# goodmattg/ndivplanning

Hardware: AMD Instinct MI355X
Metric: gan_train_steps_per_sec_traj8_batch64 (higher is better)
Workload: dtype f32; 1 GPU; BASELINE configs[1]: train_gan.py step (D update + G update), codes mode, batch=64 trajectories per GPU, traj_len=8, num_sample=6, noise_dim=2; rows_per_gpu=2688, global_batch=64, parallelism=dp1, hip_graph=True, steps_per_graph_launch=16, repeats=1, gradient_exchange=none

## Files before the change

### ndivplanning_amd/csrc/ndp_kernels.hip

```cpp
#include <hip/hip_runtime.h>
#include <math.h>
#include <stddef.h>
#include <stdint.h>

#include "ndp_device.h"

namespace ndp {

#ifdef NDP_STAMPS
__device__ unsigned long long* g_stamps = nullptr;
__device__ int g_stamp_kernel = 0;
#define NDP_STAMP_ON(id) (g_stamps != nullptr && (g_stamp_kernel == 0 || g_stamp_kernel == (id)))
#define NDP_STAMP_DECL __shared__ unsigned long long stamp_store_[64]; unsigned long long* stamp_lds_ = stamp_store_
#define NDP_STAMP_PTR stamp_lds_
#define NDP_STAMP(i)                                             \
  do {                                                           \
    if (threadIdx.x == 0) {                                      \
      stamp_lds_[2 * (i)] = clock64();                           \
      stamp_lds_[2 * (i) + 1] = wall_clock64();                  \
    }                                                            \
  } while (0)
#define NDP_STAMP_FLUSH(n, id)                                                              \
  do {                                                                                      \
    if (threadIdx.x == 0 && NDP_STAMP_ON(id))                                               \
// ... 845 lines not shown
      if (row < a.m)
        if constexpr (WT) stg4_wt(a.action_hat + row0 * 4, 4 * threadIdx.x, *reinterpret_cast<const f32x4*>(A + threadIdx.x * 4));
        else *reinterpret_cast<f32x4*>(a.action_hat + row * 4) = *reinterpret_cast<const f32x4*>(A + threadIdx.x * 4);
    }
    __syncthreads();
    NDP_STAMP(9);
    phase_a_d_part<PK, RG, NR>(a, false, tile, ntiles, dw1, dw2, CPD, XC, XT, B1, B2, L, DL, W4S, NDP_STAMP_PTR);
  } else {
    const int tile = (int)blockIdx.x - ntiles;
    const int64_t row0 = (int64_t)tile * R;
    dw1.preload(PK ? d.pf1 : d.w1 + ADIM, 260, d.b1, d.w1, ADIM);
    W4S[threadIdx.x] = d.w4[threadIdx.x];
    if (threadIdx.x == 0) W4S[256] = d.b4[0];
    for (int idx = threadIdx.x; idx < R * 64; idx += kThreads) {
      const int i = idx >> 6, k = 4 * (idx & 63);
      const int64_t row = row0 + i;
      f32x4 v = {0.f, 0.f, 0.f, 0.f};
      if (row < a.flat) v = *reinterpret_cast<const f32x4*>(a.code + row * CODE + k);
      *reinterpret_cast<f32x4*>(XC + i * 260 + k) = v;
    }
    for (int idx = threadIdx.x; idx < R * TAILLD; idx += kThreads) {
      const int i = idx / TAILLD, t = idx % TAILLD;
      const int64_t row = row0 + i;
      XT[idx] = (row < a.flat && t < ADIM) ? a.actions[row * ADIM + t] : 0.f;
    }
    __syncthreads();
    phase_a_d_part<PK, RG, 0>(a, true, tile, ntiles, dw1, dw2, nullptr, XC, XT, B1, B2, L, DL, W4S, NDP_STAMP_PTR);
  }
  (void)red;
  NDP_STAMP(8);
  NDP_STAMP_FLUSH(32, 5);
}

struct PhaseBArgs {
  GNet g; DNet d;
  const float* code; int code_rep;
  const float* action_hat;
  const float* nd_grad;
  int64_t m;
  float inv_m;
  const float *gh1, *gh2, *gh3, *gh4;
  float *dy1, *dy2, *dy3, *dy4, *dy5;
  float* loss_partials;
  float* dy1seg; int seg_s, seg_entries;
};

constexpr int phase_b_lds_floats(bool pre) {
  return 16 * (260 + TAILLD + 132 + 68 + 132 + 4 + 2) + 8 + 256 + kSW4 + kSW5 + (pre ? 16 * (260 + 132 + 68) : 0);
}

template <bool PK, int RG, bool PRE, int NR>
__global__ __launch_bounds__(kThreads, (RG >= 96 ? 2 : 3)) void k_phase_b(PhaseBArgs a_segment) {
  constexpr bool DD = NR > 0;
  constexpr int NRR = NR > 0 ? NR : 1;
  constexpr bool WT = wt_tiles(RG);
  const PhaseBArgs a = RG >= 96 ? load_kernargs<PhaseBArgs>() : a_segment;
  constexpr int R = 16;
  extern __shared__ __attribute__((aligned(16))) float smem[];
  float* XC = smem;
  float* XT = XC + R * 260;
  float* B1 = XT + R * TAILLD;
  float* B2 = B1 + R * 132;
  float* H1 = B2 + R * 68;
  float* DA = H1 + R * 132;
  float* L = DA + R * 4;
  float* DL = L + R;
  float* red = DL + R;
  float* W1A = red + 8;
  float* W4S = W1A + 256;
  float* W5S = W4S + kSW4;
  float* G4 = PRE ? W5S + kSW5 : XC;
  float* G3 = PRE ? G4 + R * 260 : B1;
  float* G2 = PRE ? G3 + R * 132 : B2;
  const int64_t row0 = (int64_t)blockIdx.x * R;
  const GNet& g = a.g;
  const DNet& d = a.d;
  NDP_STAMP_DECL;
  NDP_STAMP(0);

  FwdW<256, 64, 4, PK, RG> dw1;
  FwdW<64, 128, 4, PK, RG> dw2;
  f32x4 ct[R * 64 / kThreads];
  float av = 0.f;
  {
    if (DD) {
      load_code_rows<NRR>(XC, a.code, row0 / a.code_rep, (a.m + a.code_rep - 1) / a.code_rep);
    } else {
#pragma unroll
      for (int u = 0; u < R * 64 / kThreads; ++u) {
        const int idx = threadIdx.x + u * kThreads;
        const int i = idx >> 6, k = 4 * (idx & 63);
        const int64_t row = row0 + i;
        const bool ok = row < a.m;
        const f32x4 v = *reinterpret_cast<const f32x4*>(a.code + ((ok ? row : 0) / a.code_rep) * CODE + k);
        ct[u] = ok ? v : f32x4{0.f, 0.f, 0.f, 0.f};
      }
    }
    const int i = threadIdx.x / TAILLD, t = threadIdx.x % TAILLD;
    const int64_t row = row0 + i;
    if (row < a.m && t < ADIM) av = a.action_hat[row * ADIM + t];
  }
  const float w1a = d.w1[(threadIdx.x >> 2) * 260 + (threadIdx.x & 3)], w4r = d.w4[threadIdx.x], b4r = d.b4[0];
  const f32x4 w5r = *reinterpret_cast<const f32x4*>(g.w5 + 4 * threadIdx.x);
  pin_vmem();
  if (DD) dw2.preload(PK ? d.pf2 : d.w2, 64, d.b2, nullptr, 0);
  else dw1.preload(PK ? d.pf1 : d.w1 + ADIM, 260, d.b1, d.w1, ADIM);
  if (!DD) {
#pragma unroll
    for (int u = 0; u < R * 64 / kThreads; ++u) {
      const int idx = threadIdx.x + u * kThreads;
      *reinterpret_cast<f32x4*>(XC + (idx >> 6) * 260 + 4 * (idx & 63)) = ct[u];
    }
  }
  XT[threadIdx.x] = av;
  TileRegs<1, 128> t1;
  TileRegs<1, 256> t4;
  TileRegs<1, 128> t3;
  TileRegs<1, 64> t2;
  W1A[threadIdx.x] = w1a;
  W4S[threadIdx.x] = w4r;
  if (threadIdx.x == 0) W4S[256] = b4r;
  *reinterpret_cast<f32x4*>(W5S + 4 * threadIdx.x) = w5r;
  if (PRE) {
    t1.load(a.gh1 + row0 * 128, 128);
    t4.load(a.gh4 + row0 * 256, 256);
    t3.load(a.gh3 + row0 * 128, 128);
    t2.load(a.gh2 + row0 * 64, 64);
    pin_vmem();
  } else {
    load_tile<1, 128>(H1, 132, a.gh1 + row0 * 128, 128);
  }
  __syncthreads();
  NDP_STAMP(1);
  if (DD) {
    code_rows_dot<64, NRR>(d.pf1, XC, XC + NRR * 260);
    __syncthreads();
    fc1_from_code_rows<64, ACT_LRELU, NRR>(XC + NRR * 260, d.b1, d.w1, 260, ADIM, XT, B2, 68,
                                           (int)(row0 % a.code_rep), a.code_rep);
  } else {
    dw2.bind(PK ? d.pf2 : d.w2, 64, d.b2, nullptr, 0);
    layer_fwd_run<1, 256, 64, ACT_LRELU, 4, PK>(dw1, XC, 260, B2, 68, XT, TAILLD, dw2);
  }
  if (PRE) {
    t1.store(H1, 132);
    t4.store(G4, 260);
    t3.store(G3, 132);
    t2.store(G2, 68);
  }
  __syncthreads();
  FwdW<128, 256, 4, PK, RG> dw3;
  dw3.bind(PK ? d.pf3 : d.w3, 128, d.b3, nullptr, 0);
  layer_fwd_run<1, 64, 128, ACT_LRELU, 4, PK>(dw2, B2, 68, B1, 132, nullptr, 0, dw3);
  __syncthreads();
  DgW<128, 256, PK, RG> dg3;
  dg3.bind(PK ? d.pg3 : d.w3, 128);
  layer_fwd_run<1, 128, 256, ACT_LRELU, 4, PK>(dw3, B1, 132, XC, 260, nullptr, 0, dg3);
  __syncthreads();
  NDP_STAMP(2);
  layer_fwd_narrow<1, 256, 1>(XC, 260, W4S, W4S + 256, L, 1);
  __syncthreads();
  float lsum = 0.f;
  if (threadIdx.x < R) {
    const int64_t row = row0 + threadIdx.x;
    const float x = L[threadIdx.x];
    float dl = 0.f;
    if (row < a.m) {
      lsum = fmaxf(x, 0.f) - x + log1pf(expf(-fabsf(x)));
      dl = (1.f / (1.f + expf(-x)) - 1.f) * a.inv_m;
    }
    DL[threadIdx.x] = dl;
  }
  if (threadIdx.x < 64) {
    const float tot = wave_sum(lsum);
    if (threadIdx.x == 0) a.loss_partials[blockIdx.x] = tot;
  }
  __syncthreads();
  NDP_STAMP(3);
  layer_dgrad_narrow<1, 256, 1, ACT_LRELU>(DL, 1, W4S, XC, 260);
  __syncthreads();
  DgW<64, 128, PK, RG> dg2;
  dg2.bind(PK ? d.pg2 : d.w2, 64);
  layer_dgrad_run<1, 128, 256, ACT_LRELU, PK>(dg3, XC, 260, B1, 132, dg2);
  __syncthreads();
  DgW<128, 256, PK, RG> gg4;
  gg4.bind(PK ? g.pg4 : g.w4, 128);
  layer_dgrad_run<1, 64, 128, ACT_LRELU, PK>(dg2, B1, 132, B2, 68, gg4);
  __syncthreads();
  NDP_STAMP(4);
  {
    const int i = threadIdx.x >> 4, j = (threadIdx.x >> 2) & 3, part = threadIdx.x & 3;
    const int64_t row = row0 + i;
    const float ng = (part == 0 && row < a.m && a.nd_grad != nullptr) ? a.nd_grad[row * ADIM + j] : 0.f;
    float s = 0.f;
#pragma unroll
    for (int o = 16 * part; o < 16 * part + 16; ++o) s = fmaf(B2[i * 68 + o], W1A[o * 4 + j], s);
    s += __shfl_xor(s, 1, 64);
    s += __shfl_xor(s, 2, 64);
    if (part == 0) {
      s = row < a.m ? s + ng : 0.f;
      DA[i * ADIM + j] = s;
      a.dy5[row * ADIM + j] = s;
    }
  }
  __syncthreads();
  NDP_STAMP(5);

  if (!PRE) {
    load_tile<1, 256>(G4, 260, a.gh4 + row0 * 256, 256);
    load_tile<1, 128>(G3, 132, a.gh3 + row0 * 128, 128);
    load_tile<1, 64>(G2, 68, a.gh2 + row0 * 64, 64);
    __syncthreads();
  }
  NDP_STAMP(6);
  layer_dgrad_narrow<1, 256, 4, ACT_RELU>(DA, 4, W5S, G4, 260);
  __syncthreads();
  NDP_STAMP(7);
  DgW<64, 128, PK, RG> gg3;
  gg3.bind(PK ? g.pg3 : g.w3, 64);
  layer_dgrad_run<1, 128, 256, ACT_RELU, PK>(gg4, G4, 260, G3, 132, gg3);
  __syncthreads();
  NDP_STAMP(8);
  DgW<128, 64, PK, RG> gg2;
  gg2.bind(PK ? g.pg2 : g.w2, 128);
  store_tile<1, 256, WT>(a.dy4 + row0 * 256, 256, G4, 260);
  layer_dgrad_run<1, 64, 128, ACT_RELU, PK>(gg3, G3, 132, G2, 68, gg2);
  __syncthreads();
  NDP_STAMP(9);
  store_tile<1, 128, WT>(a.dy3 + row0 * 128, 128, G3, 132);
  layer_dgrad_run<1, 128, 64, ACT_RELU, PK>(gg2, G2, 68, H1, 132);
  __syncthreads();
  NDP_STAMP(10);
  store_tile<1, 64, WT>(a.dy2 + row0 * 64, 64, G2, 68);
  store_tile<1, 128, WT>(a.dy1 + row0 * 128, 128, H1, 132);
  store_segment_sums<128, 1>(H1, 132, a.dy1seg, row0, a.code_rep, a.seg_s, a.seg_entries, (int)blockIdx.x, (int)gridDim.x);
  NDP_STAMP(11);
  NDP_STAMP_FLUSH(12, 6);
}

__device__ __forceinline__ void adam_advance(int32_t* state, float lr, float b1, float b2) {
  const int32_t t = state[0] + 1;
  state[0] = t;
  const double bc1 = 1.0 - pow((double)b1, (double)t);
  const double bc2 = 1.0 - pow((double)b2, (double)t);
  reinterpret_cast<float*>(state)[1] = (float)((double)lr / bc1);
  reinterpret_cast<float*>(state)[2] = (float)sqrt(bc2);
}

enum { WG_FULL = 0, WG_SKINNY_B = 1, WG_SKINNY_A = 2, WG_WIDE = 3 };
constexpr int kWgradPrefetch = 8;

struct WgradJob {
  const float* A;
  const float* B;
  int lda, ldb;
  int a_cols, b_cols;
  int b_rowmod, b_rowdiv, b_rowmax;
  int b_vec;
  int dst_off, dst_ld;
  int bias_off;
  int kind;
  int rows, seg, seg_s, seg_k;
  int seg_wrap;
  int nchunks;
};
constexpr int kMaxJobs = 28;
struct WgradHead {
  int njobs;
  int nwide;
  int wide_chunks;
  int rows;
  float* slabs;
  int64_t slab_stride;
  int32_t* bump;
  float lr, beta1, beta2;
  int nchunks;
  NdivArgs nd;
};
struct WgradArgs : WgradHead {
  WgradJob job[kMaxJobs];
  int net_is_g;
  int nreg, reg_begin[4], reg_end[4];
  int wide_begin, wide_end;
};

__host__ __device__ __forceinline__ void wgrad_slot(int njobs, int nwide, int wide_chunks, int block, int& job, int& chunk) {
  const int wide_blocks = nwide * wide_chunks;
  if (block < wide_blocks) {
    job = njobs + block / wide_chunks;
    chunk = block % wide_chunks;
  } else {
    const int b = block - wide_blocks;
    const int idx = b >> 3;
    job = idx % njobs;
    chunk = (b & 7) + 8 * (idx / njobs);
  }
}

#ifdef NDP_STAMPS
#define NDP_WSTAMP(i) do { if (threadIdx.x == 0) { wst[2 * (i)] = clock64(); wst[2 * (i) + 1] = wall_clock64(); } } while (0)
#else
#define NDP_WSTAMP(i) do { } while (0)
#endif

template <int MT, int NT, int KIND, bool WT>
__device__ __forceinline__ void wgrad_block(const WgradJob& jb, int rbeg, int rend, int row_last,
                                            float* slab, float* smem, unsigned long long* wst) {
  const int lane = threadIdx.x & 63, wave = threadIdx.x >> 6;
  const int c = lane & 15, q = lane >> 4;
  f32x4 acc[MT][NT];
  float bs[MT];
#pragma unroll
  for (int u = 0; u < MT; ++u) {
    bs[u] = 0.f;
#pragma unroll
    for (int v = 0; v < NT; ++v) acc[u][v] = f32x4{0.f, 0.f, 0.f, 0.f};
  }
  constexpr int PF = kWgradPrefetch;
  const bool seg_b = jb.seg != 0;
  const bool plain_b = !seg_b && jb.b_rowdiv == 1 && jb.b_rowmod == 0x7fffffff;
  const float b_inv = 1.0f / (float)(seg_b ? jb.seg_k : jb.b_rowdiv);
  const float s_inv = 1.0f / (float)(seg_b ? jb.seg_s : 1);
  const int nsteps = rend > rbeg ? (rend - rbeg) >> 4 : 0;
  const int row_first = rbeg + 4 * wave + q;
  const int ca = KIND == WG_SKINNY_A ? (c < jb.a_cols ? c : jb.a_cols - 1) : 4 * c;
  const int cb = KIND == WG_SKINNY_B ? (c < jb.b_cols ? c : jb.b_cols - 1) : 4 * c;
  const bool a_on = KIND != WG_SKINNY_A || c < jb.a_cols;
  const bool b_on = KIND != WG_SKINNY_B || c < jb.b_cols;
  f32x4 ra[PF], rb[PF];
  auto load_a = [&](int t) -> f32x4 {
    int row = row_first + 16 * t;
    row = row < row_last ? row : row_last;
    const float* p = jb.A + (size_t)row * jb.lda + ca;
    if (KIND == WG_SKINNY_A) {
      const float v = *p;
      return f32x4{a_on ? v : 0.f, 0.f, 0.f, 0.f};
    }
    return *reinterpret_cast<const f32x4*>(p);
  };
  auto load_b = [&](int t) -> f32x4 {
    int row = row_first + 16 * t;
    row = row < row_last ? row : row_last;
    int brow = row;
    if (seg_b) {
      const bool ident = jb.seg_wrap != 0 && row >= jb.seg_wrap;
      const int e = ident ? 0 : row;
      int tile = (int)((float)e * s_inv);
      tile = tile * jb.seg_s > e ? tile - 1 : tile;
      tile = (tile + 1) * jb.seg_s <= e ? tile + 1 : tile;
      const int x = 16 * tile;
      int f0 = (int)((float)x * b_inv);
      f0 = f0 * jb.seg_k > x ? f0 - 1 : f0;
      f0 = (f0 + 1) * jb.seg_k <= x ? f0 + 1 : f0;
      brow = ident ? row - jb.seg_wrap : f0 + (e - tile * jb.seg_s);
    } else if (!plain_b) {
      const int x = row >= jb.b_rowmod ? row - jb.b_rowmod : row;
      int qd = (int)((float)x * b_inv);
      qd = qd * jb.b_rowdiv > x ? qd - 1 : qd;
      qd = (qd + 1) * jb.b_rowdiv <= x ? qd + 1 : qd;
      brow = qd;
    }
    brow = brow < jb.b_rowmax ? brow : jb.b_rowmax;
    const float* p = jb.B + (size_t)brow * jb.ldb + cb;
    if (KIND == WG_SKINNY_B) {
      const float v = *p;
      return f32x4{b_on ? v : 0.f, 0.f, 0.f, 0.f};
    }
    if (jb.b_vec) return *reinterpret_cast<const f32x4*>(p);
    return f32x4{p[0], p[1], p[2], p[3]};
  };
  auto mma_step = [&](const f32x4& va, const f32x4& vb) {
#pragma unroll
    for (int u = 0; u < MT; ++u) {
      bs[u] += va[u];
#pragma unroll
      for (int v = 0; v < NT; ++v) acc[u][v] = mfma16(va[u], vb[v], acc[u][v]);
    }
  };
  NDP_WSTAMP(1);
#pragma unroll
  for (int p = 0; p < PF; ++p) {
    ra[p] = load_a(p);
    rb[p] = load_b(p);
  }
  pin_vmem();
  int t = 0;
  for (; t + PF <= nsteps; t += PF) {
#pragma unroll
    for (int p = 0; p < PF; ++p) {
      const f32x4 va = ra[p], vb = rb[p];
      ra[p] = load_a(t + p + PF);
      rb[p] = load_b(t + p + PF);
      pin_vmem();
      mma_step(va, vb);
    }
  }
  const int rem = nsteps - t;
#pragma unroll
  for (int p = 0; p < PF; ++p)
    if (p < rem) mma_step(ra[p], rb[p]);
  NDP_WSTAMP(2);
  constexpr int JR = KIND == WG_SKINNY_A ? 16 : 64;
  constexpr int KC = KIND == WG_SKINNY_B ? 16 : 64;
  float* mine = smem + wave * (JR * KC);
  float* bsh = smem + kWaves * (JR * KC);
#pragma unroll
  for (int u = 0; u < MT; ++u)
#pragma unroll
    for (int i = 0; i < 4; ++i) {
      const int j = KIND == WG_SKINNY_A ? (4 * q + i) : (4 * (4 * q + i) + u);
      if (KIND == WG_SKINNY_B) {
        mine[j * KC + c] = acc[u][0][i];
      } else {
        f32x4 t;
#pragma unroll
        for (int v = 0; v < NT; ++v) t[v] = acc[u][v][i];
        *reinterpret_cast<f32x4*>(mine + j * KC + 4 * c) = t;
      }
    }
#pragma unroll
  for (int u = 0; u < MT; ++u) {
    float s = bs[u];
    s += __shfl_xor(s, 16, 64);
    s += __shfl_xor(s, 32, 64);
    if (q == 0) bsh[wave * 64 + (KIND == WG_SKINNY_A ? c : 4 * c + u)] = s;
  }
  __syncthreads();
  NDP_WSTAMP(3);
  const int jn = jb.a_cols, kn = jb.b_cols;
  for (int e = threadIdx.x; e < JR * KC / 4; e += kThreads) {
    const int j = e / (KC / 4), k = 4 * (e % (KC / 4));
    f32x4 s = *reinterpret_cast<const f32x4*>(smem + j * KC + k);
#pragma unroll
    for (int w = 1; w < kWaves; ++w) s += *reinterpret_cast<const f32x4*>(smem + w * (JR * KC) + j * KC + k);
    if (j < jn) {
      float* d = slab + jb.dst_off + (size_t)j * jb.dst_ld + k;
      if (KIND != WG_SKINNY_B && ((jb.dst_ld | jb.dst_off) & 3) == 0) {
        if constexpr (WT) stg4_wt(slab + jb.dst_off, (uint32_t)(j * jb.dst_ld + k), s);
        else *reinterpret_cast<f32x4*>(d) = s;
      } else {
#pragma unroll
        for (int t = 0; t < 4; ++t)
          if (k + t < kn) d[t] = s[t];
      }
    }
  }
  if (jb.bias_off >= 0 && threadIdx.x < 64 && (int)threadIdx.x < jn) {
    const int j = threadIdx.x;
    slab[jb.bias_off + j] = bsh[j] + bsh[64 + j] + bsh[128 + j] + bsh[192 + j];
  }
}

constexpr int kWideR = 16;
constexpr int wide_slab_floats() { return kWideR * (128 + 128); }
constexpr int wgrad_wide_lds_floats() { return 3 * wide_slab_floats(); }
template <bool WT>
__device__ __forceinline__ void wgrad_wide(const WgradJob& jb, int rbeg, int rend, float* slab, float* smem) {
  typedef __attribute__((address_space(3))) void* lds_ptr_t;
  typedef const __attribute__((address_space(1))) void* glb_ptr_t;
  constexpr int AW = 128;
  constexpr int SLAB = wide_slab_floats();
  const int t = threadIdx.x, lane = t & 63, wave = t >> 6;
  const int c = lane & 15, q = lane >> 4;
  const int jt = wave >> 1, kt0 = wave & 1;
  f32x4 acc[4][4];
  float bs[4];
#pragma unroll
  for (int u = 0; u < 4; ++u) {
    bs[u] = 0.f;
#pragma unroll
    for (int v = 0; v < 4; ++v) acc[u][v] = f32x4{0.f, 0.f, 0.f, 0.f};
  }
  const int nslabs = rend > rbeg ? (rend - rbeg) / kWideR : 0;
  auto fetch = [&](int s) {
    float* buf = smem + (s % 3) * SLAB;
    const size_t r0 = (size_t)rbeg + (size_t)s * kWideR;
#pragma unroll
    for (int i = 0; i < 2; ++i) {
      const int pair = wave + 4 * i;
      __builtin_amdgcn_global_load_lds((glb_ptr_t)(jb.A + (r0 + 2 * pair + (lane >> 5)) * jb.lda + 4 * (lane & 31)),
                                       (lds_ptr_t)(buf + pair * 256), 16, 0, 0);
    }
#pragma unroll
    for (int i = 0; i < 2; ++i) {
      const int pair = wave + 4 * i;
      __builtin_amdgcn_global_load_lds((glb_ptr_t)(jb.B + (r0 + 2 * pair + (lane >> 5)) * jb.ldb + 4 * (lane & 31)),
                                       (lds_ptr_t)(buf + kWideR * AW + pair * 256), 16, 0, 0);
    }
  };
  if (nslabs > 0) fetch(0);
  if (nslabs > 1) fetch(1);
  for (int s = 0; s < nslabs; ++s) {
    if (s + 1 < nslabs) asm volatile("s_waitcnt vmcnt(4)" ::: "memory");
    else asm volatile("s_waitcnt vmcnt(0)" ::: "memory");
    __builtin_amdgcn_s_barrier();
    if (s + 2 < nslabs) fetch(s + 2);
    const float* As = smem + (s % 3) * SLAB + 64 * jt + 4 * c;
    const float* Bs = smem + (s % 3) * SLAB + kWideR * AW + 64 * kt0 + 4 * c;
#pragma unroll
    for (int st = 0; st < kWideR / 4; ++st) {
      const f32x4 va = *reinterpret_cast<const f32x4*>(As + (4 * st + q) * AW);
      const f32x4 vb = *reinterpret_cast<const f32x4*>(Bs + (4 * st + q) * 128);
#pragma unroll
      for (int u = 0; u < 4; ++u) {
        if (kt0 == 0) bs[u] += va[u];
#pragma unroll
        for (int v = 0; v < 4; ++v) acc[u][v] = mfma16(va[u], vb[v], acc[u][v]);
      }
    }
  }
#pragma unroll
  for (int u = 0; u < 4; ++u)
#pragma unroll
    for (int i = 0; i < 4; ++i) {
      const f32x4 o = {acc[u][0][i], acc[u][1][i], acc[u][2][i], acc[u][3][i]};
      if constexpr (WT) {
        stg4_wt(slab + jb.dst_off, (uint32_t)((64 * jt + 4 * (4 * q + i) + u) * jb.dst_ld + 64 * kt0 + 4 * c), o);
      } else {
        float* d = slab + jb.dst_off + (size_t)(64 * jt + 4 * (4 * q + i) + u) * jb.dst_ld + 64 * kt0 + 4 * c;
        *reinterpret_cast<f32x4*>(d) = o;
      }
    }
  if (jb.bias_off >= 0 && kt0 == 0) {
#pragma unroll
    for (int u = 0; u < 4; ++u) {
      float sum = bs[u];
      sum += __shfl_xor(sum, 16, 64);
      sum += __shfl_xor(sum, 32, 64);
      if (q == 0) slab[jb.bias_off + 64 * jt + 4 * c + u] = sum;
    }
  }
}

constexpr int wgrad_lds_floats() { return kWaves * 64 * 64 + kWaves * 64; }
constexpr int wgrad_wide_launch_lds_floats() { return wgrad_wide_lds_floats() > wgrad_lds_floats() ? wgrad_wide_lds_floats() : wgrad_lds_floats(); }

__device__ __forceinline__ void wgrad_fetch_args(WgradHead& a, WgradJob& jb, int& job_id, int& chunk) {
  typedef const __attribute__((address_space(4))) char* kbytes_t;
  static_assert(sizeof(WgradHead) <= 192 && offsetof(WgradArgs, job) % 8 == 0, "k_wgrad argument prefetch");
    kbytes_t kp = (kbytes_t)__builtin_amdgcn_kernarg_segment_ptr();
    uint32_t h0, h1, h2, hw0, hw1;
    asm volatile("s_load_dword %0, %5, 0x0\n\ts_load_dword %1, %5, 0x40\n\ts_load_dword %2, %5, 0x80\n\t"
                 "s_load_dword %3, %5, 0x4\n\ts_load_dword %4, %5, 0x8\n\ts_waitcnt lgkmcnt(0)"
                 : "=&s"(h0), "=&s"(h1), "=&s"(h2), "=&s"(hw0), "=&s"(hw1) : "s"(kp) : "memory");
    wgrad_slot((int)h0, (int)hw0, (int)hw1, (int)blockIdx.x, job_id, chunk);
    const uint32_t joff = (uint32_t)(offsetof(WgradArgs, job) + (size_t)job_id * sizeof(WgradJob));
    uint32_t j0, j1;
    asm volatile("s_load_dword %0, %2, %3\n\ts_load_dword %1, %2, %4\n\ts_waitcnt lgkmcnt(0)"
                 : "=&s"(j0), "=&s"(j1) : "s"(kp), "s"(joff), "s"(joff + (uint32_t)sizeof(WgradJob) - 4u) : "memory");
    uint64_t v = (uint64_t)kp;
    asm volatile("" : "+s"(v) : "s"(h0 | h1 | h2 | j0 | j1));
    __builtin_memcpy(&a, (kbytes_t)v, sizeof(WgradHead));
    __builtin_memcpy(&jb, (kbytes_t)v + joff, sizeof(WgradJob));
}

template <bool WIDE>
__device__ __forceinline__ void wgrad_body(float* smem) {
  WgradHead a;
  WgradJob jb;
  int job_id, chunk;
  wgrad_fetch_args(a, jb, job_id, chunk);
  const int slots = a.nwide * a.wide_chunks + 8 * ((a.nchunks + 7) / 8) * a.njobs;
  if ((int)blockIdx.x >= slots) {
    ndiv_block<4, 2>(a.nd, (int)blockIdx.x - slots, smem);
    return;
  }
  if (chunk >= jb.nchunks) return;
  const int jrows = jb.rows != 0 ? jb.rows : a.rows;
  const int jrpc = ((jrows + jb.nchunks - 1) / jb.nchunks + 15) & ~15;
  const int rbeg = chunk * jrpc;
  int rend = rbeg + jrpc;
  rend = rend < jrows ? rend : jrows;
  float* slab = a.slabs + (size_t)chunk * a.slab_stride;
  if (a.bump != nullptr && blockIdx.x == 0 && threadIdx.x == 0)
    adam_advance(a.bump, a.lr, a.beta1, a.beta2);
  const int kind = jb.kind;
#ifdef NDP_STAMPS
  __shared__ unsigned long long wst[32];
  NDP_WSTAMP(0);
#else
  unsigned long long* wst = nullptr;
#endif
  constexpr bool WT = WIDE ? kWtSlabsWide : kWtSlabs;
  if (WIDE && kind == WG_WIDE) wgrad_wide<WT>(jb, rbeg, rend, slab, smem);
  else if (kind == WG_FULL) wgrad_block<4, 4, WG_FULL, WT>(jb, rbeg, rend, jrows - 1, slab, smem, wst);
  else if (kind == WG_SKINNY_B) wgrad_block<4, 1, WG_SKINNY_B, WT>(jb, rbeg, rend, jrows - 1, slab, smem, wst);
  else wgrad_block<1, 4, WG_SKINNY_A, WT>(jb, rbeg, rend, jrows - 1, slab, smem, wst);
#ifdef NDP_STAMPS
  NDP_WSTAMP(4);
  if (threadIdx.x == 0 && NDP_STAMP_ON(4))
    for (int i_ = 0; i_ < 10; ++i_) g_stamps[(size_t)blockIdx.x * 64 + i_] = wst[i_];
#endif
}

__global__ __launch_bounds__(kThreads) void k_wgrad(WgradArgs a_segment) {
  extern __shared__ __attribute__((aligned(16))) float smem[];
  (void)a_segment;
  wgrad_body<false>(smem);
}
__global__ __launch_bounds__(kThreads, 2) void k_wgrad_wide(WgradArgs a_segment) {
  extern __shared__ __attribute__((aligned(16))) float smem[];
  (void)a_segment;
  wgrad_body<true>(smem);
}

struct LossTerm {
  const float* partials; int count; float scale; int slot;
};
constexpr int kP2PRanks = 8;
constexpr int kP2PCapD = 58368;
constexpr int kP2PCapG = 86016;
constexpr int kP2PBlocks = kP2PCapG / kThreads;
constexpr int64_t kP2PFlagOff = 64;
constexpr int64_t kP2PInboxD = kP2PFlagOff + 2ll * kP2PRanks * kP2PBlocks;
constexpr int64_t kP2PInboxG = kP2PInboxD + (int64_t)kP2PRanks * 2 * kP2PCapD;
constexpr int64_t kP2PWords = kP2PInboxG + (int64_t)kP2PRanks * 2 * kP2PCapG;

struct P2PArgs {
  int world, rank, net;
  long long timeout_ticks;
  uint32_t* region[kP2PRanks];
};

__device__ __forceinline__ float p2p_sum(const P2PArgs& x, float g, int64_t p, bool valid, uint32_t step) {
  const int W = x.world, me = x.rank;
  const int64_t cap = x.net == 0 ? kP2PCapD : kP2PCapG;
  const int64_t inbox = x.net == 0 ? kP2PInboxD : kP2PInboxG;
  const int64_t par = (int64_t)(step & 1u) * cap;
  if (valid) {
    const int64_t at = inbox + (int64_t)me * 2 * cap + par + p;
#pragma unroll
    for (int r = 0; r < kP2PRanks; ++r)
      if (r < W && r != me)
        __hip_atomic_store(reinterpret_cast<float*>(x.region[r]) + at, g, __ATOMIC_RELAXED, __HIP_MEMORY_SCOPE_SYSTEM);
  }
  __builtin_amdgcn_fence(__ATOMIC_RELEASE, "workgroup");
  asm volatile("s_waitcnt vmcnt(0)" ::: "memory");
  __syncthreads();
  const int t = threadIdx.x;
  if (t < W && t != me) {
    const int64_t fbase = kP2PFlagOff + (int64_t)x.net * kP2PRanks * kP2PBlocks + blockIdx.x;
    __hip_atomic_store(x.region[t] + fbase + (int64_t)me * kP2PBlocks, step, __ATOMIC_RELAXED, __HIP_MEMORY_SCOPE_SYSTEM);
    uint32_t* status = x.region[me];
    const uint32_t* flag = x.region[me] + fbase + (int64_t)t * kP2PBlocks;
    if (__hip_atomic_load(status, __ATOMIC_RELAXED, __HIP_MEMORY_SCOPE_SYSTEM) == 0u) {
      const long long t0 = wall_clock64();
      while ((int32_t)(__hip_atomic_load(flag, __ATOMIC_RELAXED, __HIP_MEMORY_SCOPE_SYSTEM) - step) < 0) {
        if (wall_clock64() - t0 > x.timeout_ticks) {
          const uint32_t seen = __hip_atomic_load(flag, __ATOMIC_RELAXED, __HIP_MEMORY_SCOPE_SYSTEM);
          uint32_t expected = 0u;
          if (__hip_atomic_compare_exchange_strong(status, &expected, (uint32_t)(1 + t), __ATOMIC_RELAXED,
                                                   __ATOMIC_RELAXED, __HIP_MEMORY_SCOPE_SYSTEM)) {
            __hip_atomic_store(status + 1, (uint32_t)blockIdx.x, __ATOMIC_RELAXED, __HIP_MEMORY_SCOPE_SYSTEM);
            __hip_atomic_store(status + 2, (uint32_t)x.net, __ATOMIC_RELAXED, __HIP_MEMORY_SCOPE_SYSTEM);
            __hip_atomic_store(status + 3, step, __ATOMIC_RELAXED, __HIP_MEMORY_SCOPE_SYSTEM);
            __hip_atomic_store(status + 4, seen, __ATOMIC_RELAXED, __HIP_MEMORY_SCOPE_SYSTEM);
            __hip_atomic_store(status + 5, (uint32_t)t, __ATOMIC_RELAXED, __HIP_MEMORY_SCOPE_SYSTEM);
            __hip_atomic_store(status + 6, (uint32_t)(wall_clock64() - t0), __ATOMIC_RELAXED, __HIP_MEMORY_SCOPE_SYSTEM);
          }
          break;
        }
        __builtin_amdgcn_s_sleep(2);
      }
    }
  }
  __syncthreads();
  float v[kP2PRanks];
  const float* own = reinterpret_cast<const float*>(x.region[me]) + inbox + par + p;
#pragma unroll
  for (int r = 0; r < kP2PRanks; ++r)
    v[r] = __hip_atomic_load(own + (int64_t)(r < W ? r : me) * 2 * cap, __ATOMIC_RELAXED, __HIP_MEMORY_SCOPE_SYSTEM);
  float s = 0.f;
#pragma unroll
  for (int r = 0; r < kP2PRanks; ++r)
    if (r < W) s += (r == me) ? g : v[r];
  (void)valid;
  return s;
}

struct ReduceHot {
  const float* slabs; int64_t slab_stride; int64_t n;
  float *params, *exp_avg, *exp_avg_sq;
  const int32_t* step;
  float* grad;
  int nchunks, nregions; int reg_begin[4], reg_end[4], reg_slabs[4];
  float beta1, beta2, eps, lr;
};
struct ReduceArgs : ReduceHot {
  int nloss; LossTerm loss[3];
  float* losses; float* loss_sums;
  PackSpec pack;
  P2PArgs p2p;
};

__device__ __forceinline__ void adam_update(float& p, float g, float& m, float& v,
                                            float step_size, float bc2_sqrt, float b1, float b2, float eps) {
  m = __builtin_fmaf(g - m, 1.f - b1, m);
  v = __builtin_fmaf(v, b2, (1.f - b2) * g * g);
  const float denom = sqrtf(v) / bc2_sqrt + eps;
  p = __builtin_fmaf(-step_size, m / denom, p);
}

struct ReduceLossArgs { int nloss; LossTerm loss[3]; float* losses; float* loss_sums; };
// ... 118 lines not shown
```

Measured before the change: 13390 steps/s.

## Specialize wgrad inner loop per B row-mapping mode with pointer-increment addressing

Moves the weight-gradient accumulation loop into a templated helper that is instantiated separately for the plain, divided, segmented and segmented-wrap B row mappings, so runtime branching on the mapping mode leaves the inner loop. For plain mapping, A and B addresses are advanced by pointer increments with clamping instead of recomputing row indices each step. The loop now issues the MFMAs before the next loads, fenced by sched_barrier, and the skinny masking moves into the MMA step. Costs: B loads are always four scalar loads because the b_vec vector path is gone, and skinny kinds are always treated as plain mapping.

```diff
diff --git a/ndivplanning_amd/csrc/ndp_kernels.hip b/ndivplanning_amd/csrc/ndp_kernels.hip
--- a/ndivplanning_amd/csrc/ndp_kernels.hip
+++ b/ndivplanning_amd/csrc/ndp_kernels.hip
@@ -1171,6 +1171,111 @@
 #define NDP_WSTAMP(i) do { } while (0)
 #endif
 
+enum { WB_PLAIN = 0, WB_DIV = 1, WB_SEG = 2, WB_SEGWRAP = 3 };
+
+template <int MT, int NT, int KIND, int BMAP>
+__device__ __forceinline__ void wgrad_loop(const WgradJob& jb, int rbeg, int rend, int row_last,
+                                           f32x4 (&acc)[MT][NT], float (&bs)[MT]) {
+  const int lane = threadIdx.x & 63, wave = threadIdx.x >> 6;
+  const int c = lane & 15, q = lane >> 4;
+  constexpr int PF = kWgradPrefetch;
+  constexpr bool SEG = BMAP == WB_SEG || BMAP == WB_SEGWRAP;
+  const float b_inv = 1.0f / (float)(SEG ? jb.seg_k : jb.b_rowdiv);
+  const float s_inv = 1.0f / (float)(SEG ? jb.seg_s : 1);
+  const int nsteps = rend > rbeg ? (rend - rbeg) >> 4 : 0;
+  const int row_first = rbeg + 4 * wave + q;
+  const int ca = KIND == WG_SKINNY_A ? (c < jb.a_cols ? c : jb.a_cols - 1) : 4 * c;
+  const int cb = KIND == WG_SKINNY_B ? (c < jb.b_cols ? c : jb.b_cols - 1) : 4 * c;
+  const bool a_on = KIND != WG_SKINNY_A || c < jb.a_cols;
+  const bool b_on = KIND != WG_SKINNY_B || c < jb.b_cols;
+  f32x4 ra[PF], rb[PF];
+  const int b_last = row_last < jb.b_rowmax ? row_last : jb.b_rowmax;
+  const float* pa = jb.A + (size_t)(row_first < row_last ? row_first : row_last) * jb.lda + ca;
+  const float* const pa_last = jb.A + (size_t)row_last * jb.lda + ca;
+  const size_t a_step = (size_t)16 * jb.lda, b_step = (size_t)16 * jb.ldb;
+  const float* pb = jb.B + (size_t)(row_first < b_last ? row_first : b_last) * jb.ldb + cb;
+  const float* const pb_last = jb.B + (size_t)b_last * jb.ldb + cb;
+  int nrow = row_first;
+  auto b_row = [&](int r) -> int {
+    int row = r < row_last ? r : row_last;
+    int brow;
+    if (SEG) {
+      int ident = BMAP == WB_SEGWRAP && row >= jb.seg_wrap ? -1 : 0;
+      if (BMAP == WB_SEGWRAP) asm("" : "+v"(ident));
+      const int e = row & ~ident;
+      int tile = (int)((float)e * s_inv);
+      tile = tile * jb.seg_s > e ? tile - 1 : tile;
+      tile = (tile + 1) * jb.seg_s <= e ? tile + 1 : tile;
+      const int x = 16 * tile;
+      int f0 = (int)((float)x * b_inv);
+      f0 = f0 * jb.seg_k > x ? f0 - 1 : f0;
+      f0 = (f0 + 1) * jb.seg_k <= x ? f0 + 1 : f0;
+      brow = ((row - jb.seg_wrap) & ident) | ((f0 + (e - tile * jb.seg_s)) & ~ident);
+    } else {
+      const int x = row >= jb.b_rowmod ? row - jb.b_rowmod : row;
+      int qd = (int)((float)x * b_inv);
+      qd = qd * jb.b_rowdiv > x ? qd - 1 : qd;
+      qd = (qd + 1) * jb.b_rowdiv <= x ? qd + 1 : qd;
+      brow = qd;
+    }
+    return brow < jb.b_rowmax ? brow : jb.b_rowmax;
+  };
+  if (BMAP != WB_PLAIN) pb = jb.B + (size_t)b_row(nrow) * jb.ldb + cb;
+  auto advance = [&]() {
+    const float* na = pa + a_step;
+    pa = (uintptr_t)na < (uintptr_t)pa_last ? na : pa_last;
+    if (BMAP == WB_PLAIN) {
+      const float* nb = pb + b_step;
+      pb = (uintptr_t)nb < (uintptr_t)pb_last ? nb : pb_last;
+    } else {
+      nrow += 16;
+      pb = jb.B + (size_t)b_row(nrow) * jb.ldb + cb;
+    }
+  };
+  auto load_a = [&]() -> f32x4 {
+    if (KIND == WG_SKINNY_A) return f32x4{*pa, 0.f, 0.f, 0.f};
+    return *reinterpret_cast<const f32x4*>(pa);
+  };
+  auto load_b = [&]() -> f32x4 {
+    if (KIND == WG_SKINNY_B) return f32x4{*pb, 0.f, 0.f, 0.f};
+    return f32x4{pb[0], pb[1], pb[2], pb[3]};
+  };
+  auto mma_step = [&](f32x4 va, f32x4 vb) {
+    if (KIND == WG_SKINNY_A) va[0] = a_on ? va[0] : 0.f;
+    if (KIND == WG_SKINNY_B) vb[0] = b_on ? vb[0] : 0.f;
+#pragma unroll
+    for (int u = 0; u < MT; ++u) {
+      bs[u] += va[u];
+#pragma unroll
+      for (int v = 0; v < NT; ++v) acc[u][v] = mfma16(va[u], vb[v], acc[u][v]);
+      asm volatile("" : "+v"(bs[u]));
+    }
+  };
+#pragma unroll
+  for (int p = 0; p < PF; ++p) {
+    ra[p] = load_a();
+    rb[p] = load_b();
+    advance();
+  }
+  __builtin_amdgcn_sched_barrier(0);
+  int t = 0;
+  for (; t + PF <= nsteps; t += PF) {
+#pragma unroll
+    for (int p = 0; p < PF; ++p) {
+      mma_step(ra[p], rb[p]);
+      __builtin_amdgcn_sched_barrier(0);
+      ra[p] = load_a();
+      rb[p] = load_b();
+      __builtin_amdgcn_sched_barrier(0);
+      advance();
+    }
+  }
+  const int rem = nsteps - t;
+#pragma unroll
+  for (int p = 0; p < PF; ++p)
+    if (p < rem) mma_step(ra[p], rb[p]);
+}
+
 template <int MT, int NT, int KIND, bool WT>
 __device__ __forceinline__ void wgrad_block(const WgradJob& jb, int rbeg, int rend, int row_last,
                                             float* slab, float* smem, unsigned long long* wst) {
@@ -1184,89 +1289,17 @@
 #pragma unroll
     for (int v = 0; v < NT; ++v) acc[u][v] = f32x4{0.f, 0.f, 0.f, 0.f};
   }
-  constexpr int PF = kWgradPrefetch;
-  const bool seg_b = jb.seg != 0;
-  const bool plain_b = !seg_b && jb.b_rowdiv == 1 && jb.b_rowmod == 0x7fffffff;
-  const float b_inv = 1.0f / (float)(seg_b ? jb.seg_k : jb.b_rowdiv);
-  const float s_inv = 1.0f / (float)(seg_b ? jb.seg_s : 1);
-  const int nsteps = rend > rbeg ? (rend - rbeg) >> 4 : 0;
-  const int row_first = rbeg + 4 * wave + q;
-  const int ca = KIND == WG_SKINNY_A ? (c < jb.a_cols ? c : jb.a_cols - 1) : 4 * c;
-  const int cb = KIND == WG_SKINNY_B ? (c < jb.b_cols ? c : jb.b_cols - 1) : 4 * c;
-  const bool a_on = KIND != WG_SKINNY_A || c < jb.a_cols;
-  const bool b_on = KIND != WG_SKINNY_B || c < jb.b_cols;
-  f32x4 ra[PF], rb[PF];
-  auto load_a = [&](int t) -> f32x4 {
-    int row = row_first + 16 * t;
-    row = row < row_last ? row : row_last;
-    const float* p = jb.A + (size_t)row * jb.lda + ca;
-    if (KIND == WG_SKINNY_A) {
-      const float v = *p;
-      return f32x4{a_on ? v : 0.f, 0.f, 0.f, 0.f};
-    }
-    return *reinterpret_cast<const f32x4*>(p);
-  };
-  auto load_b = [&](int t) -> f32x4 {
-    int row = row_first + 16 * t;
-    row = row < row_last ? row : row_last;
-    int brow = row;
-    if (seg_b) {
-      const bool ident = jb.seg_wrap != 0 && row >= jb.seg_wrap;
-      const int e = ident ? 0 : row;
-      int tile = (int)((float)e * s_inv);
-      tile = tile * jb.seg_s > e ? tile - 1 : tile;
-      tile = (tile + 1) * jb.seg_s <= e ? tile + 1 : tile;
-      const int x = 16 * tile;
-      int f0 = (int)((float)x * b_inv);
-      f0 = f0 * jb.seg_k > x ? f0 - 1 : f0;
-      f0 = (f0 + 1) * jb.seg_k <= x ? f0 + 1 : f0;
-      brow = ident ? row - jb.seg_wrap : f0 + (e - tile * jb.seg_s);
-    } else if (!plain_b) {
-      const int x = row >= jb.b_rowmod ? row - jb.b_rowmod : row;
-      int qd = (int)((float)x * b_inv);
-      qd = qd * jb.b_rowdiv > x ? qd - 1 : qd;
-      qd = (qd + 1) * jb.b_rowdiv <= x ? qd + 1 : qd;
-      brow = qd;
-    }
-    brow = brow < jb.b_rowmax ? brow : jb.b_rowmax;
-    const float* p = jb.B + (size_t)brow * jb.ldb + cb;
-    if (KIND == WG_SKINNY_B) {
-      const float v = *p;
-      return f32x4{b_on ? v : 0.f, 0.f, 0.f, 0.f};
-    }
-    if (jb.b_vec) return *reinterpret_cast<const f32x4*>(p);
-    return f32x4{p[0], p[1], p[2], p[3]};
-  };
-  auto mma_step = [&](const f32x4& va, const f32x4& vb) {
-#pragma unroll
-    for (int u = 0; u < MT; ++u) {
-      bs[u] += va[u];
-#pragma unroll
-      for (int v = 0; v < NT; ++v) acc[u][v] = mfma16(va[u], vb[v], acc[u][v]);
-    }
-  };
   NDP_WSTAMP(1);
-#pragma unroll
-  for (int p = 0; p < PF; ++p) {
-    ra[p] = load_a(p);
-    rb[p] = load_b(p);
-  }
-  pin_vmem();
-  int t = 0;
-  for (; t + PF <= nsteps; t += PF) {
-#pragma unroll
-    for (int p = 0; p < PF; ++p) {
-      const f32x4 va = ra[p], vb = rb[p];
-      ra[p] = load_a(t + p + PF);
-      rb[p] = load_b(t + p + PF);
-      pin_vmem();
-      mma_step(va, vb);
-    }
-  }
-  const int rem = nsteps - t;
-#pragma unroll
-  for (int p = 0; p < PF; ++p)
-    if (p < rem) mma_step(ra[p], rb[p]);
+#define NDP_WGRAD_LOOP(BMAP) wgrad_loop<MT, NT, KIND, BMAP>(jb, rbeg, rend, row_last, acc, bs)
+  if (KIND == WG_FULL) {
+    const int bmap = jb.seg != 0 ? (jb.seg_wrap != 0 ? WB_SEGWRAP : WB_SEG)
+                                 : (jb.b_rowdiv == 1 && jb.b_rowmod == 0x7fffffff ? WB_PLAIN : WB_DIV);
+    if (bmap == WB_PLAIN) NDP_WGRAD_LOOP(WB_PLAIN);
+    else if (bmap == WB_DIV) NDP_WGRAD_LOOP(WB_DIV);
+    else if (bmap == WB_SEG) NDP_WGRAD_LOOP(WB_SEG);
+    else NDP_WGRAD_LOOP(WB_SEGWRAP);
+  } else NDP_WGRAD_LOOP(WB_PLAIN);
+#undef NDP_WGRAD_LOOP
   NDP_WSTAMP(2);
   constexpr int JR = KIND == WG_SKINNY_A ? 16 : 64;
   constexpr int KC = KIND == WG_SKINNY_B ? 16 : 64;
```

Measured after the change: 13650 steps/s (median of 6 runs). +1.9%, better.
